# Kim-Dongjun/Soft-Truncation

Measured on AMD Instinct MI355X. Metric: training images/sec (DDPM++ CIFAR-10 32x32), higher is better.
Workload: dtype f32; 1 GPU; DDPM++ (VP) CIFAR-10 32x32, configs/vp/CIFAR10/ddpmpp_nll_st.py (BASELINE configs[1]); per_gpu_batch=128, global_batch=128, parallelism=dp1

## Files before the change

### soft-truncation_amd/csrc/conv.hip

```cpp
#include "igemm.h"
#include "split.h"
#include "stk_fp16.h"
#include "stk_fp16_train.h"

namespace {

using igemm::Cfg;
using igemm::MnMajor;
using igemm::keep_if;
using igemm::strip_row;

typedef __attribute__((address_space(1))) float gfloat;

struct ConvP {
  const float* x1; const float* x2; int C1, C2;
  const float* w; int w_layout;
  const float* bias; const float* temb; int temb_stride; const float* res; float inv_div; int use_div;
  float* y;
  const float* dy; float* dx1; float* dx2; float beta1, beta2, alpha;
  float* part; long part_stride;
  int N, H, W, Cin, Cout, OH, OW, KH, KW, stride, pad, sshift;
  int HW, OHW, taps;
  int ohw_shift, ow_shift;
};
// ... 630 lines not shown
#pragma unroll
      for (int t = 0; t < 9; ++t) v[u][t] = src[(long)(z + u) * stride + (long)t * CC];
#pragma unroll
    for (int u = 0; u < 4; ++u)
#pragma unroll
      for (int t = 0; t < 9; ++t) acc[t] += v[u][t];
  }
  for (; z < splits; ++z)
#pragma unroll
    for (int t = 0; t < 9; ++t) acc[t] += src[(long)z * stride + (long)t * CC];
#pragma unroll
  for (int t = 0; t < 9; ++t) s[threadIdx.x * 9 + t] = alpha * acc[t];
  __syncthreads();
  const long base = q0 * 9, end = CC * 9;
#pragma unroll
  for (int k = 0; k < 9; ++k) {
    const long i = base + k * 256 + threadIdx.x;
    if (i < end) dw[i] += s[k * 256 + threadIdx.x];
  }
}

template <int COLS>
__global__ __launch_bounds__(256) void wgrad9_kernel(ConvP p, int tiles_m, int tiles_n, int k_per_split) {
  constexpr int ROWS = 32 / COLS, TW = COLS + 2, TH = ROWS + 2, TSZ = TH * TW;
  constexpr int XS = TSZ | 1;
  constexpr int LDA = 129;
  constexpr int NX = (32 * TSZ + 255) / 256;
  constexpr int NA = 16;
  __shared__ float lds[32 * LDA + 32 * XS];
  float* As = lds;
  float* Xs = lds + 32 * LDA;

  const int tid = threadIdx.x, lane = tid & 63, wid = tid >> 6;
  const int fk = lane >> 5, fc = lane & 31;
  const int id = xcd_remap(blockIdx.x, gridDim.x);
  const int tn = id % tiles_n;
  const int rest = id / tiles_n;
  const int tm = rest % tiles_m, zs = rest / tiles_m;
  const int m0 = tm * 128, n0 = tn * 32;
  const int K = p.N * p.OHW;
  const int k_begin = zs * k_per_split;
  const int k_end = min(K, k_begin + k_per_split);

  const int mrow = m0 + (tid >> 5), cout_hi = p.Cout - 1;
  unsigned okrowsA = 0;
#pragma unroll
  for (int i = 0; i < NA; ++i) okrowsA |= (mrow + 8 * i < p.Cout ? 1u : 0u) << i;
  const int cin_hi = p.Cin - 1;
  floatx16 acc[9];
#pragma unroll
  for (int t = 0; t < 9; ++t)
#pragma unroll
    for (int e = 0; e < 16; ++e) acc[t][e] = 0.f;

  float ra[NA], rx[NX];
  unsigned okmA = 0, okmX = 0;
  auto load = [&](int k0) {
    const int k = k0 + (tid & 31);
    const bool kv = k < K;
    int b, ohw;
    split_pixel(p, kv ? k : 0, b, ohw);
    const int abase = b * p.Cout * p.OHW + ohw;
    okmA = kv ? okrowsA : 0u;
#pragma unroll
    for (int i = 0; i < NA; ++i) ra[i] = p.dy[abase + min(mrow + 8 * i, cout_hi) * p.OHW];
    int b0, ohw0, oy0, ox0;
    split_pixel(p, k0, b0, ohw0);
    split_row(p, ohw0, oy0, ox0);
    const int xbase = b0 * p.Cin * p.HW + (oy0 - 1) * p.W + (ox0 - 1);
    okmX = 0;
#pragma unroll
    for (int i = 0; i < NX; ++i) {
      const int e = tid + 256 * i;
      const int ci = e / TSZ, rem = e - ci * TSZ;
      const int lr = rem / TW, lc = rem - lr * TW;
      const int iy = oy0 - 1 + lr, ix = ox0 - 1 + lc;
      const bool ok = e < 32 * TSZ && n0 + ci < p.Cin && iy >= 0 && iy < p.H && ix >= 0 && ix < p.W;
      rx[i] = p.x1[ok ? xbase + min(n0 + ci, cin_hi) * p.HW + lr * p.W + lc : 0];
      okmX |= (ok ? 1u : 0u) << i;
    }
  };
  auto store = [&]() {
#pragma unroll
    for (int i = 0; i < NA; ++i) As[(tid & 31) * LDA + (tid >> 5) + 8 * i] = keep_if(ra[i], okmA, i);
#pragma unroll
    for (int i = 0; i < NX; ++i) {
      const int e = tid + 256 * i;
      const int ci = e / TSZ, rem = e - ci * TSZ;
      if (e < 32 * TSZ) Xs[ci * XS + rem] = keep_if(rx[i], okmX, i);
    }
  };

  if (k_begin < k_end) load(k_begin);
  const float* arow = As + fk * LDA + wid * 32 + fc;
  const float* xrow = Xs + fc * XS + fk;
  for (int k0 = k_begin; k0 < k_end; k0 += 32) {
    store();
    __syncthreads();
    if (k0 + 32 < k_end) load(k0 + 32);
#pragma unroll
    for (int ks = 0; ks < 16; ++ks) {
      const float a = arow[2 * ks * LDA];
      constexpr int dummy = 0; (void)dummy;
      const int loc = ((2 * ks) / COLS) * TW + ((2 * ks) % COLS);
      float bv[9];
#pragma unroll
      for (int t = 0; t < 9; ++t) bv[t] = xrow[loc + (t / 3) * TW + (t % 3)];
#pragma unroll
      for (int t = 0; t < 9; ++t) acc[t] = __builtin_amdgcn_mfma_f32_32x32x2f32(a, bv[t], acc[t], 0, 0, 0);
    }
    __syncthreads();
  }

  float* slab = p.part + (long)zs * p.part_stride;
  const int n = n0 + fc;
  if (n < p.Cin) {
#pragma unroll
    for (int t = 0; t < 9; ++t)
#pragma unroll
      for (int e = 0; e < 16; ++e) {
        const int m = m0 + wid * 32 + strip_row(e) + 4 * fk;
        if (m < p.Cout) slab[((long)t * p.Cout + m) * p.Cin + n] = acc[t][e];
      }
  }
}

struct GemmP {
  const float* A; long sam, sak, sab;
  const float* B; long sbk, sbn, sbb;
  float* C; long scm, scn, scb;
  const float* bias; int bias_mode;
  int M, N, K;
  float alpha, beta;
};
template <class C, bool K_CONTIG>
struct GA {
  RowChunk<C::BM, C::KC, C::LDA> rc;
  MnStrided<C::BM, C::KC, C::LDA> ms;
  __device__ void init(const GemmP& p, int m0, int tid, int zb) {
    const float* base = p.A + (long)zb * p.sab;
    if (K_CONTIG) rc.init(base, p.sam, m0, p.M, p.K, tid);
    else ms.init(base, p.sam, p.sak, m0, p.M, p.K, tid);
  }
  __device__ void load(const GemmP&, int k0, float (&r)[C::NA]) {
    if (K_CONTIG) rc.load(k0, r); else ms.load(k0, r);
  }
  __device__ void store(const float (&r)[C::NA], float* t) {
    if (K_CONTIG) rc.store(r, t); else ms.store(r, t);
  }
};
template <class C, bool K_CONTIG>
struct GB {
  RowChunk<C::BN, C::KC, C::LDB> rc;
  MnStrided<C::BN, C::KC, C::LDB> ms;
  __device__ void init(const GemmP& p, int n0, int tid, int zb) {
    const float* base = p.B + (long)zb * p.sbb;
    if (K_CONTIG) rc.init(base, p.sbn, n0, p.N, p.K, tid);
    else ms.init(base, p.sbn, p.sbk, n0, p.N, p.K, tid);
  }
  __device__ void load(const GemmP&, int k0, float (&r)[C::NB]) {
    if (K_CONTIG) rc.load(k0, r); else ms.load(k0, r);
  }
  __device__ void store(const float (&r)[C::NB], float* t) {
    if (K_CONTIG) rc.store(r, t); else ms.store(r, t);
  }
};
struct EpGemm {
  float* base;
  __device__ void init(const GemmP& p, int zb, int) { base = p.C + (long)zb * p.scb; }
  __device__ void col(const GemmP&, int) {}
  __device__ void strip(const GemmP& p, int mbase, int M, bool nok, int n, const floatx16& acc) {
    float old[16];
    if (p.beta != 0.f) {
#pragma unroll
      for (int e = 0; e < 16; ++e) {
        const int m = mbase + strip_row(e);
        const bool ok = nok && m < M;
        old[e] = base[ok ? (long)m * p.scm + (long)n * p.scn : 0];
      }
    }
#pragma unroll
    for (int e = 0; e < 16; ++e) {
      const int m = mbase + strip_row(e);
      if (nok && m < M) {
        float v = p.alpha * acc[e];
        if (p.bias_mode == 1) v += p.bias[m];
        else if (p.bias_mode == 2) v += p.bias[n];
        base[(long)m * p.scm + (long)n * p.scn] = (p.beta != 0.f ? p.beta * old[e] : 0.f) + v;
      }
    }
  }
};

inline bool use_big_tile(int M, long N, int z) {
  const long t = (long)stk_cdiv(M, 128) * stk_cdiv(N, 128) * z;
  return M >= 96 && N >= 96 && t >= 192;
}

template <class C, class P, class AL, class BL, class EP>
int launch(const P& p, int M, long Nl, int K, int k_per_split, int splits, int batch, hipStream_t s,
           bool flat = false) {
  if (Nl > 0x7fffffffL) return STK_EUNSUPPORTED;
  const int N = (int)Nl;
  const int tm = stk_cdiv(M, C::BM), tn = stk_cdiv(N, C::BN);
  if (flat) {
    const long total = (long)tm * tn * splits * batch;
    if (total > 0x7fffffffL) return STK_EUNSUPPORTED;
    hipLaunchKernelGGL((igemm::kernel<C, P, AL, BL, EP>), dim3((unsigned)total), dim3(256), 0, s, p, M, N, K, tm, tn,
                       k_per_split, batch);
  } else {
    dim3 grid((unsigned)(tm * tn), (unsigned)splits, (unsigned)batch);
    hipLaunchKernelGGL((igemm::kernel<C, P, AL, BL, EP>), grid, dim3(256), 0, s, p, M, N, K, tm, tn, k_per_split, 0);
  }
  STK_CHECK_LAUNCH();
  return STK_OK;
}

inline int fill_common(ConvP& p, int N, int H, int W, int C1, int C2, int Cout, int OH, int OW, int KH, int KW,
                       int stride, int pad) {
  if (N <= 0 || H <= 0 || W <= 0 || C1 <= 0 || C2 < 0 || Cout <= 0 || OH <= 0 || OW <= 0) return STK_EINVAL;
  if (!((KH == 3 && KW == 3) || (KH == 1 && KW == 1))) return STK_EUNSUPPORTED;
  if (stride != 1 && stride != 2) return STK_EUNSUPPORTED;
  const long lim = 0x7fffffffL;
  if ((long)N * (C1 > C2 ? C1 : C2) * H * W >= lim || (long)N * Cout * OH * OW >= lim) return STK_EUNSUPPORTED;
  p.N = N; p.H = H; p.W = W; p.C1 = C1; p.C2 = C2; p.Cin = C1 + C2; p.Cout = Cout; p.OH = OH; p.OW = OW;
  p.KH = KH; p.KW = KW; p.stride = stride; p.pad = pad; p.sshift = stride == 2 ? 1 : 0;
  p.HW = H * W; p.OHW = OH * OW; p.taps = KH * KW;
  p.ohw_shift = -1; p.ow_shift = -1;
  for (int sft = 0; sft < 31; ++sft) {
    if ((1 << sft) == p.OHW) p.ohw_shift = sft;
    if ((1 << sft) == p.OW) p.ow_shift = sft;
  }
  return STK_OK;
}

struct SplitPlan { int ok; int splits; int chunks_per_split; long slab; int t64; int gps; };
inline SplitPlan split_plan(const ConvP& p, int Kc, int S1, int S2, int M, long Ng) {
  SplitPlan r = {0, 1, 0, 0, 0, 0};
  const long big = (long)p.N * p.HW * 4 * (S1 > S2 ? S1 : S2);
  const bool geom = (p.taps == 9 && p.pad == 1) || (p.taps == 1 && p.pad == 0);
  if (!(big < 0x7fffffffL && geom && p.stride == 1 && p.OH == p.H && p.OW == p.W && Kc % 32 == 0 &&
        (S2 == 0 || S1 % 32 == 0) && M >= 96 && Ng <= 0x7fffffffL))
    return r;
  const long tiles = (long)stk_cdiv(M, 128) * stk_cdiv(Ng, 128);
  const int nch = p.taps * (Kc / 32);
  r.chunks_per_split = nch;
  if (tiles >= 192) { r.ok = 1; return r; }
  static const long target = [] { const char* e = getenv("STK_KSPLIT_WGS"); return e && atol(e) > 0 ? atol(e) : 512L; }();
  constexpr long minch = 12;
  long splits = target / tiles;
  const long mc = p.taps == 9 ? minch : (minch < 6 ? minch : 6);
  if (splits > nch / mc) splits = nch / mc;
  if ((tiles < 16 && p.taps != 9) || splits < 2) return r;
  r.chunks_per_split = (int)((nch + splits - 1) / splits);
  r.splits = (nch + r.chunks_per_split - 1) / r.chunks_per_split;
  r.slab = (long)M * Ng;
  r.ok = 1;
  return r;
}
inline SplitPlan fwd_split_plan(const ConvP& p) { return split_plan(p, p.Cin, p.C1, p.C2, p.Cout, (long)p.N * p.OHW); }
inline SplitPlan dgrad_split_plan(const ConvP& p) { return split_plan(p, p.Cout, p.Cout, 0, p.Cin, (long)p.N * p.HW); }
struct SplitWs { long xpart, part, bytes; };
inline long align256(long v) { return (v + 255) & ~255L; }
inline SplitWs split_ws(const SplitPlan& r, int M, int Kc, int taps) {
  SplitWs o;
  o.xpart = align256(x2::wp_bytes(M, Kc, taps));
  o.part = align256(o.xpart + 2L * x2::NPART * 4);
  o.bytes = r.ok ? 255 + o.part + (r.splits > 1 ? r.splits * r.slab * 4 : 0) : 0;
  return o;
}
inline void split_weight_strides(const ConvP& p, int dgrad, long& sm, long& sk) {
  if (p.w_layout == 0) { sm = dgrad ? p.taps : (long)p.Cin * p.taps; sk = dgrad ? (long)p.Cin * p.taps : p.taps; }
  else { sm = dgrad ? p.Cout : 1; sk = dgrad ? 1 : p.Cout; }
}
inline SplitPlan x1_plan(const SplitPlan& r, int nch1) {
  SplitPlan r1 = r;
  r1.chunks_per_split = (nch1 + r.splits - 1) / r.splits;
  r1.splits = (nch1 + r1.chunks_per_split - 1) / r1.chunks_per_split;
  return r1;
}

struct SplitGemm {
  ConvP p; x2::Src q; int M, Ng, tm, tn, nch, chunks_per_split; const float* xpart; int nx;
  bool dual, planes, halo; dim3 grid; hipStream_t s;
};
template <class E, int TAPS>
void split_gemm_taps(const SplitGemm& g) {
  constexpr bool X1 = is_x1<E>::value;
  if (!g.planes) {
    using A1 = std::conditional_t<X1, x2::ActLoader16<false, TAPS>, x2::ActLoader<false, TAPS>>;
    using A2 = std::conditional_t<X1, x2::ActLoader16<true, TAPS>, x2::ActLoader<true, TAPS>>;
    if (g.dual) hipLaunchKernelGGL((x2::gemm_kernel<A2, E>), g.grid, dim3(256), 0, g.s, g.p, g.q, g.M, g.Ng, g.tm, g.tn, g.nch,
                                   g.chunks_per_split, g.xpart, g.nx);
    else hipLaunchKernelGGL((x2::gemm_kernel<A1, E>), g.grid, dim3(256), 0, g.s, g.p, g.q, g.M, g.Ng, g.tm, g.tn, g.nch,
                            g.chunks_per_split, g.xpart, g.nx);
  } else if (g.halo) {
    if (g.p.W == 64)
      hipLaunchKernelGGL((x2d::gemm_halo_kernel<64, E, 1>), g.grid, dim3(256), 0, g.s, g.p, g.q, g.M, g.Ng, g.tm, g.tn, g.nch / 9, g.xpart, g.nx);
    else if (g.p.W == 32)
      hipLaunchKernelGGL((x2d::gemm_halo_kernel<32, E, 1>), g.grid, dim3(256), 0, g.s, g.p, g.q, g.M, g.Ng, g.tm, g.tn, g.nch / 9, g.xpart, g.nx);
    else
      hipLaunchKernelGGL((x2d::gemm_halo_kernel<16, E, 1>), g.grid, dim3(256), 0, g.s, g.p, g.q, g.M, g.Ng, g.tm, g.tn, g.nch / 9, g.xpart, g.nx);
  } else {
    hipLaunchKernelGGL((x2d::gemm_kernel<TAPS, 128, E>), g.grid, dim3(256), 0, g.s, g.p, g.q, g.M, g.Ng, g.tm, g.tn, g.nch,
                       g.chunks_per_split, g.xpart, g.nx);
  }
}
template <class E>
void split_gemm(const SplitGemm& g) {
  if (g.p.taps == 9) split_gemm_taps<E, 9>(g);
  else split_gemm_taps<E, 1>(g);
}

template <class EP>
int launch_split(ConvP p, const SplitPlan& r0, const float* s1, int S1, const float* s2, int S2, int M, long Ng, int dgrad,
                 void* ws, hipStream_t s, const void* wp_ready, float* amax, const void* planes, const float* planes_amax,
                 bool amax_valid, bool x1) {
  x2::Src q;
  q.s1 = s1; q.s2 = S2 > 0 ? s2 : s1; q.S1 = S1; q.S2 = S2; q.Kc = S1 + S2; q.Mpad = x2::pad128(M); q.taps = p.taps;
  q.pl = static_cast<const unsigned char*>(planes); q.pl_stride = planes ? pl::plane_bytes(p.N, S1, p.HW) : 0;
  const SplitWs lay = split_ws(r0, M, q.Kc, p.taps);
  unsigned char* base = reinterpret_cast<unsigned char*>(((uintptr_t)ws + 255) & ~(uintptr_t)255);
  float* xpart = reinterpret_cast<float*>(base + lay.xpart);
  p.part = reinterpret_cast<float*>(base + lay.part);
  p.part_stride = r0.slab;
  if (amax) xpart = amax + (dgrad ? 2 * x2::NPART : 0);
  if (planes) {
    xpart = const_cast<float*>(planes_amax);
  } else if (!(amax_valid && amax)) {
    hipLaunchKernelGGL(x2::amax_partial_kernel, dim3(x2::NPART), dim3(x2::AMAX_THREADS), 0, s, s1, (long)p.N * S1 * p.HW, xpart);
    if (S2 > 0)
      hipLaunchKernelGGL(x2::amax_partial_kernel, dim3(x2::NPART), dim3(x2::AMAX_THREADS), 0, s, s2, (long)p.N * S2 * p.HW,
                         xpart + x2::NPART);
    STK_CHECK_LAUNCH();
  }
  if (wp_ready) {
    q.wp = static_cast<const unsigned short*>(wp_ready);
  } else {
    x2::WprepDesc one = {};
    one.w = p.w; one.wp = base; one.M = M; one.Kc = q.Kc; one.Mpad = q.Mpad;
    one.taps = p.taps; one.flip = dgrad;
    split_weight_strides(p, dgrad, one.sm, one.sk);
    hipLaunchKernelGGL(x2::wamax_kernel, dim3(x2::WPART, 1), dim3(256), 0, s, nullptr, one);
    hipLaunchKernelGGL(x2::wprep_kernel, dim3((unsigned)stk_cdiv((long)q.Mpad * q.Kc, 256L)), dim3(256), 0, s, nullptr, one);
    STK_CHECK_LAUNCH();
    q.wp = reinterpret_cast<const unsigned short*>(base);
  }
  const int nch = planes && x1 ? p.taps * ((q.Kc / x2::KC + 1) / 2) : p.taps * (q.Kc / x2::KC);
  const SplitPlan r = planes && x1 ? x1_plan(r0, nch) : r0;
  SplitGemm g = {p, q, M, (int)Ng, q.Mpad / 128, stk_cdiv((int)Ng, 128), nch, r.chunks_per_split, xpart,
                 S2 > 0 ? 2 * x2::NPART : x2::NPART, S2 > 0, planes != nullptr, planes && x2d::halo_ok(p, p.taps, r0.splits),
                 dim3(), s};
  g.grid = dim3((unsigned)(g.tm * g.tn * r.splits));
  if (r0.splits == 1) {
    if (x1) split_gemm<OneProduct<EP>>(g);
    else split_gemm<EP>(g);
    STK_CHECK_LAUNCH();
    return STK_OK;
  }
  if (x1) split_gemm<OneProduct<EpSlab>>(g);
  else split_gemm<EpSlab>(g);
  STK_CHECK_LAUNCH();
  launch_slab_sum(p, r.splits, M, Ng, dgrad, s);
  STK_CHECK_LAUNCH();
  return STK_OK;
}

struct SplitWgradPlan { int ok; int splits; int chunks_per_split; long slab; int rows3; };
inline SplitWgradPlan split_wgrad_plan(int C1, int C2, int N, int Cout, int H, int W, int OH, int OW, int KH, int KW,
                                       int stride, int pad) {
  SplitWgradPlan q = {0, 0, 0, 0, 0};
  const int Cin = C1 + C2;
  const long K = (long)N * H * W;
  const int cmax = Cout > C1 ? (Cout > C2 ? Cout : C2) : (C1 > C2 ? C1 : C2);
  if (K * cmax * 4 >= 0x7fffffffL || (C2 > 0 && C1 % 32)) return q;
  const bool pow2 = (W & (W - 1)) == 0 && ((H * W) & (H * W - 1)) == 0;
  const bool geom = (KH == 3 && KW == 3 && pad == 1) || (KH == 1 && KW == 1 && pad == 0);
  if (!geom || stride != 1 || OH != H || OW != W || !pow2 || W < 4 || H * W < 16 || Cin < 64 || Cout < 64 ||
      K > 0x7fffffffL || K % 32)
    return q;
  const int taps = KH * KW;
  q.rows3 = (taps == 9 && W >= 8 && (C2 == 0 || C1 % 16 == 0)) ? 1 : 0;
  const long tiles = q.rows3 ? 3L * stk_cdiv(Cout, 128) * stk_cdiv(Cin, 64)
                             : (long)taps * stk_cdiv(Cout, 128) * stk_cdiv(Cin, 128);
  if (taps == 1 && tiles < 2) return q;
  const long chunks = K / 32;
  constexpr long w1_wgs = 256;
  long splits = (taps == 1 && tiles < 6 ? w1_wgs : 512) / tiles;
  if (splits > chunks / 8) splits = chunks / 8;
  if (splits < 1) splits = 1;
  q.chunks_per_split = (int)((chunks + splits - 1) / splits);
  q.splits = (int)((chunks + q.chunks_per_split - 1) / q.chunks_per_split);
  q.slab = (long)Cout * Cin * taps;
  q.ok = 1;
  return q;
}
template <int FORM>
void launch_x2w(const x2w::Args& a, int W, dim3 grid, hipStream_t s) {
  const dim3 block(256 * (FORM & 15));
  if (W >= 32) hipLaunchKernelGGL((x2w::wgrad_kernel<32, FORM>), grid, block, 0, s, a);
  else if (W == 16) hipLaunchKernelGGL((x2w::wgrad_kernel<16, FORM>), grid, block, 0, s, a);
  else if (W == 8) hipLaunchKernelGGL((x2w::wgrad_kernel<8, FORM>), grid, block, 0, s, a);
  else hipLaunchKernelGGL((x2w::wgrad_kernel<4, FORM>), grid, block, 0, s, a);
}
struct WgemmArgs {
  ConvP p; int tm, tn, nch, chunks_per_split; const float* dyp; const float* xp; int nx; dim3 grid; hipStream_t s;
};
template <bool X1, class BL>
void launch_wgemm_rows(const WgemmArgs& g) {
  using AL = std::conditional_t<X1, x2::RowsU16<false, false>, x2::RowsU<false, false>>;
  using E = std::conditional_t<X1, OneProduct<EpWgrad>, EpWgrad>;
  hipLaunchKernelGGL((x2::wgemm_kernel<AL, BL, E, !X1>), g.grid, dim3(256), 0, g.s, g.p, g.p.Cout, g.p.Cin, g.tm, g.tn, g.nch,
                     g.chunks_per_split, g.p.taps, g.dyp, g.xp, g.nx);
}
template <bool X1, bool DUAL>
void launch_wgemm_src(const WgemmArgs& g) {
  if (g.p.taps == 1)
    launch_wgemm_rows<X1, std::conditional_t<X1, x2::RowsU16<true, DUAL>, x2::RowsU<true, DUAL>>>(g);
  else if (g.p.W >= 16)
    launch_wgemm_rows<X1, std::conditional_t<X1, x2::RowsB16<DUAL, 16>, x2::RowsB<DUAL, 16>>>(g);
  else if (g.p.W == 8)
    launch_wgemm_rows<X1, std::conditional_t<X1, x2::RowsB16<DUAL, 8>, x2::RowsB<DUAL, 8>>>(g);
  else
    launch_wgemm_rows<X1, std::conditional_t<X1, x2::RowsB16<DUAL, 4>, x2::RowsB<DUAL, 4>>>(g);
}
template <bool X1>
void launch_wgemm(const WgemmArgs& g) {
  if (g.p.C2 > 0) launch_wgemm_src<X1, true>(g);
  else launch_wgemm_src<X1, false>(g);
}

struct WgradPlan { int big; int splits; int k_per_split; long slab; int mode9; };
inline int wgrad9_cols(int OH, int OW, int KH, int KW) {
  if (KH != 3 || KW != 3 || ((long)OH * OW) % 32 != 0) return 0;
  if (OW % 32 == 0) return 32;
  if (OW == 16 || OW == 8) return OW;
  return 0;
}
inline WgradPlan wgrad_plan(int Cin, int N, int Cout, int OH, int OW, int KH, int KW, bool allow9 = true) {
  WgradPlan q;
  q.mode9 = allow9 ? wgrad9_cols(OH, OW, KH, KW) : 0;
  if (q.mode9) {
    const long K = (long)N * OH * OW;
    const long tiles = (long)stk_cdiv(Cout, 128) * stk_cdiv(Cin, 32);
    const long chunks = K / 32;
    long splits = 256 / tiles;
    if (splits > chunks / 16) splits = chunks / 16;
    if (splits < 1) splits = 1;
    const long cps = (chunks + splits - 1) / splits;
    q.big = 1;
    q.k_per_split = (int)(cps * 32);
    q.splits = (int)((K + q.k_per_split - 1) / q.k_per_split);
    q.slab = (long)Cout * Cin * 9;
    return q;
  }
  const int taps = KH * KW;
  const long K = (long)N * OH * OW;
  const long tiles128 = (long)stk_cdiv(Cout, 128) * stk_cdiv(Cin, 128) * taps;
  q.big = (Cout >= 96 && Cin >= 96 && tiles128 >= 9) ? 1 : 0;
  const int T = q.big ? 128 : 64;
  const long tiles = (long)stk_cdiv(Cout, T) * stk_cdiv(Cin, T) * taps;
  const long chunks = (K + 31) / 32;
  long splits = (512 + tiles - 1) / tiles;
  if (splits > chunks / 16) splits = chunks / 16;
  if (splits < 1) splits = 1;
  const long cps = (chunks + splits - 1) / splits;
  q.k_per_split = (int)(cps * 32);
  q.splits = (int)((K + q.k_per_split - 1) / q.k_per_split);
  q.slab = (long)Cout * Cin * taps;
  return q;
}

}

extern "C" {

static int fwd_impl(const float* x1, int C1, const float* x2, int C2, const float* w, int w_layout,
                    const float* bias, const float* temb, int temb_stride, const float* res, float out_div,
                    float* y, int N, int H, int W, int Cout, int OH, int OW, int KH, int KW, int stride, int pad,
                    const void* wp, float* amax, void* ws, long ws_bytes, void* stream, bool x_rec_valid, bool f16x1) {
  if (!x1 || !w || !y || (C2 > 0 && !x2) || out_div == 0.f || (w_layout != 0 && w_layout != 1) ||
      (w_layout == 1 && (KH != 1 || KW != 1)))
    return STK_EINVAL;
  ConvP p = {};
  int rc = fill_common(p, N, H, W, C1, C2, Cout, OH, OW, KH, KW, stride, pad);
  if (rc) return rc;
  p.x1 = x1; p.x2 = C2 > 0 ? x2 : x1; p.w = w; p.w_layout = w_layout; p.bias = bias; p.temb = temb;
  p.temb_stride = temb_stride; p.res = res; p.inv_div = 1.f / out_div; p.use_div = out_div != 1.f; p.y = y;
  const int K = p.Cin * p.taps;
  const long Ng = (long)N * p.OHW;
  const bool big = use_big_tile(Cout, Ng, 1);
  hipStream_t s = (hipStream_t)stream;
  if (thin::geometry_ok(p) && Ng <= 0x7fffffffL) {
    const unsigned nblk = (unsigned)stk_cdiv(Ng, 256L);
    if (C2 == 0 && p.Cin <= 4) {
      thin::Args a = {x1, w, (long)p.Cin * p.taps, (long)p.taps, 0, p.Cin, Cout, p.taps, 0};
      const dim3 grid(nblk, (unsigned)stk_cdiv(Cout, thin::OB));
      if (p.taps == 9) hipLaunchKernelGGL((thin::thin_in_kernel<9>), grid, dim3(256), 0, s, p, a);
      else hipLaunchKernelGGL((thin::thin_in_kernel<1>), grid, dim3(256), 0, s, p, a);
      STK_CHECK_LAUNCH();
      return STK_OK;
    }
    if (Cout <= 4) {
      const unsigned nblk64 = (unsigned)stk_cdiv(Ng, 64L);
      if (p.taps == 9) hipLaunchKernelGGL((thin::thin_out_kernel<9>), dim3(nblk64), dim3(256), 0, s, p, Cout);
      else hipLaunchKernelGGL((thin::thin_out_kernel<1>), dim3(nblk64), dim3(256), 0, s, p, Cout);
      STK_CHECK_LAUNCH();
      return STK_OK;
    }
  }
  const SplitPlan xr = fwd_split_plan(p);
  if (ws && xr.ok && ws_bytes >= split_ws(xr, Cout, p.Cin, p.taps).bytes)
    return launch_split<EpFwd>(p, xr, x1, C1, x2, C2, Cout, Ng, 0, ws, s, wp, amax, nullptr, nullptr, x_rec_valid, f16x1);
  if (wp) return STK_EINVAL;
  if (p.taps == 9) {
    using CB = Cfg<128, 128, 36>; using CS = Cfg<64, 64, 36>;
    if (C2 > 0) {
      if (big) return launch<CB, ConvP, AFwdK<CB>, BFwd<CB, 9, true>, EpFwd>(p, Cout, Ng, K, K, 1, 1, s);
      return launch<CS, ConvP, AFwdK<CS>, BFwd<CS, 9, true>, EpFwd>(p, Cout, Ng, K, K, 1, 1, s);
    }
    if (big) return launch<CB, ConvP, AFwdK<CB>, BFwd<CB, 9, false>, EpFwd>(p, Cout, Ng, K, K, 1, 1, s);
    return launch<CS, ConvP, AFwdK<CS>, BFwd<CS, 9, false>, EpFwd>(p, Cout, Ng, K, K, 1, 1, s);
  }
  using CB = Cfg<128, 128, 32>; using CS = Cfg<64, 64, 32>;
  if (w_layout == 0) {
    if (K % 8 == 0) {
      if (big) return launch<CB, ConvP, AFwdK<CB>, BFwd<CB, 1, true>, EpFwd>(p, Cout, Ng, K, K, 1, 1, s);
      return launch<CS, ConvP, AFwdK<CS>, BFwd<CS, 1, true>, EpFwd>(p, Cout, Ng, K, K, 1, 1, s);
    }
    return launch<CS, ConvP, AFwdGen<CS>, BFwd<CS, 1, true>, EpFwd>(p, Cout, Ng, K, K, 1, 1, s);
  }
  if (big) return launch<CB, ConvP, AFwdNin<CB>, BFwd<CB, 1, true>, EpFwd>(p, Cout, Ng, K, K, 1, 1, s);
  return launch<CS, ConvP, AFwdNin<CS>, BFwd<CS, 1, true>, EpFwd>(p, Cout, Ng, K, K, 1, 1, s);
}

int stk_conv2d_fwd_f32(const float* x1, int C1, const float* x2, int C2, const float* w, int w_layout,
                       const float* bias, const float* temb, int temb_stride, const float* res, float out_div,
                       float* y, int N, int H, int W, int Cout, int OH, int OW, int KH, int KW, int stride, int pad,
                       void* ws, long ws_bytes, void* stream) {
  return stk_conv2d_fwd_wp_f32(x1, C1, x2, C2, w, w_layout, bias, temb, temb_stride, res, out_div, y, N, H, W, Cout, OH, OW,
                               KH, KW, stride, pad, nullptr, nullptr, ws, ws_bytes, stream);
}

int stk_conv2d_fwd_wp_f32(const float* x1, int C1, const float* x2, int C2, const float* w, int w_layout,
                          const float* bias, const float* temb, int temb_stride, const float* res, float out_div,
                          float* y, int N, int H, int W, int Cout, int OH, int OW, int KH, int KW, int stride, int pad,
                          const void* wp, float* amax, void* ws, long ws_bytes, void* stream) {
  return fwd_impl(x1, C1, x2, C2, w, w_layout, bias, temb, temb_stride, res, out_div, y, N, H, W, Cout, OH, OW, KH, KW, stride,
                  pad, wp, amax, ws, ws_bytes, stream, false, false);
}

int stk_conv2d_fwd_rec_f32(const float* x1, int C1, const float* x2, int C2, const float* w, int w_layout,
                           const float* bias, const float* temb, int temb_stride, const float* res, float out_div,
                           float* y, int N, int H, int W, int Cout, int OH, int OW, int KH, int KW, int stride, int pad,
                           const void* wp, float* amax, void* ws, long ws_bytes, void* stream) {
  if (!amax) return STK_EINVAL;
  return fwd_impl(x1, C1, x2, C2, w, w_layout, bias, temb, temb_stride, res, out_div, y, N, H, W, Cout, OH, OW, KH, KW, stride,
                  pad, wp, amax, ws, ws_bytes, stream, true, false);
}

int stk_conv2d_fwd_wp_f16x1(const float* x1, int C1, const float* x2, int C2, const float* w, int w_layout,
                            const float* bias, const float* temb, int temb_stride, const float* res, float out_div,
                            float* y, int N, int H, int W, int Cout, int OH, int OW, int KH, int KW, int stride, int pad,
                            const void* wp, float* amax, void* ws, long ws_bytes, void* stream) {
  return fwd_impl(x1, C1, x2, C2, w, w_layout, bias, temb, temb_stride, res, out_div, y, N, H, W, Cout, OH, OW, KH, KW, stride,
                  pad, wp, amax, ws, ws_bytes, stream, false, true);
}

int stk_conv2d_fwd_rec_f16x1(const float* x1, int C1, const float* x2, int C2, const float* w, int w_layout,
                             const float* bias, const float* temb, int temb_stride, const float* res, float out_div,
                             float* y, int N, int H, int W, int Cout, int OH, int OW, int KH, int KW, int stride, int pad,
                             const void* wp, float* amax, void* ws, long ws_bytes, void* stream) {
  if (!amax) return STK_EINVAL;
  return fwd_impl(x1, C1, x2, C2, w, w_layout, bias, temb, temb_stride, res, out_div, y, N, H, W, Cout, OH, OW, KH, KW, stride,
                  pad, wp, amax, ws, ws_bytes, stream, true, true);
}

static int dgrad_impl(const float* dy, const float* w, int w_layout, float* dx1, int C1, float beta1, float* dx2,
                      int C2, float beta2, float alpha, int N, int H, int W, int Cout, int OH, int OW, int KH,
                      int KW, int stride, int pad, const void* wp, float* amax, void* ws, long ws_bytes,
                      void* stream, bool dy_rec_valid, bool f16x1) {
  if (!dy || !w || (!dx1 && !dx2) || (w_layout != 0 && w_layout != 1) || (w_layout == 1 && (KH != 1 || KW != 1)))
    return STK_EINVAL;
  ConvP p = {};
  int rc = fill_common(p, N, H, W, C1, C2, Cout, OH, OW, KH, KW, stride, pad);
  if (rc) return rc;
  p.dy = dy; p.w = w; p.w_layout = w_layout; p.dx1 = dx1; p.dx2 = C2 > 0 ? dx2 : nullptr;
  p.beta1 = beta1; p.beta2 = beta2; p.alpha = alpha;
  const int Cin = p.Cin;
  const int K = Cout * p.taps;
  const long Ng = (long)N * p.HW;
  const bool big = use_big_tile(Cin, Ng, 1);
  hipStream_t s = (hipStream_t)stream;
  if (thin::geometry_ok(p) && Cout <= 4 && Ng <= 0x7fffffffL) {
    thin::Args a = {dy, w, (long)p.taps, (long)Cin * p.taps, 1, Cout, Cin, p.taps, 1};
    const dim3 grid((unsigned)stk_cdiv(Ng, 256L), (unsigned)stk_cdiv(Cin, thin::OB));
    if (p.taps == 9) hipLaunchKernelGGL((thin::thin_in_kernel<9>), grid, dim3(256), 0, s, p, a);
    else hipLaunchKernelGGL((thin::thin_in_kernel<1>), grid, dim3(256), 0, s, p, a);
    STK_CHECK_LAUNCH();
    return STK_OK;
  }
  const SplitPlan xr = dgrad_split_plan(p);
  if (ws && xr.ok && ws_bytes >= split_ws(xr, Cin, Cout, p.taps).bytes)
    return launch_split<EpDgrad>(p, xr, dy, Cout, nullptr, 0, Cin, Ng, 1, ws, s, wp, amax, nullptr, nullptr, dy_rec_valid, f16x1);
  if (wp) return STK_EINVAL;
  if (p.taps == 9) {
    using CB = Cfg<128, 128, 36>; using CS = Cfg<64, 64, 36>;
    if (big) return launch<CB, ConvP, ADgrad9<CB>, BDgrad<CB, 9>, EpDgrad>(p, Cin, Ng, K, K, 1, 1, s);
// ... 464 lines not shown
```

### soft-truncation_amd/csrc/conv_x2d.h

```cpp
#pragma once

namespace x2d {

using x2::KC;
typedef __attribute__((address_space(3))) void lds_void;

template <int TN>
struct Geo {
  static constexpr int A_PLANE = 128 * 64, A_BYTES = 2 * A_PLANE;
  static constexpr int B_PLANE = TN * 64, B_BYTES = 2 * B_PLANE;
  static constexpr int LDS = A_BYTES + B_BYTES;
  static constexpr int NJ = TN / 64;
  static constexpr int BBLK = TN / 64;
};

__device__ __forceinline__ void dma16(__amdgpu_buffer_rsrc_t rs, unsigned char* dst, unsigned voff, unsigned soff) {
  __builtin_amdgcn_raw_ptr_buffer_load_lds(rs, (lds_void*)dst, 16, (int)voff, (int)soff, 0, 0);
}

template <int TAPS, int TN, class EP, int NBUF = 1, int ABL = 0>
__global__ __launch_bounds__(256, 2) void gemm_kernel(ConvP p, x2::Src q, int M, int Nn, int tiles_m, int tiles_n,
                                                      int nchunks_total, int chunks_per_split,
                                                      const float* __restrict__ xpart, int nxpart) {
  using G = Geo<TN>;
  constexpr bool X1 = is_x1<EP>::value;
  __shared__ __attribute__((aligned(1024))) unsigned char lds[G::LDS * NBUF];
  unsigned char* const As = lds;
  unsigned char* const Bs = lds + G::A_BYTES;
  const int tid = threadIdx.x;
  const int lane = tid & 63, wid = __builtin_amdgcn_readfirstlane(tid >> 6);
  __shared__ float red_amax[4];
  x2::LateAmax xmax;
  xmax.load(xpart, nxpart, tid);
  const float sw = x2::weight_scale(q.wp);
  const int ntiles = tiles_m * tiles_n;
  const int id = xcd_remap(blockIdx.x, gridDim.x);
  const int tile = id % ntiles, zs = id / ntiles;
  const int tm = tile % tiles_m, tn = tile / tiles_m;
  const int m0 = tm * 128, n0 = tn * TN;
  const int c_begin = zs * chunks_per_split;
  const int c_last = min(nchunks_total, c_begin + chunks_per_split) - 1;

  const unsigned seg_src = (unsigned)((lane & 3) ^ ((lane >> 4) & 3)) * 16u;
  const unsigned a_plane2 = (unsigned)q.taps * q.Mpad * q.Kc * 2u;
  const unsigned a_chunk2 = (unsigned)q.Mpad * KC * 2u;
  const __amdgpu_buffer_rsrc_t a_rs = x2::make_rsrc(reinterpret_cast<const unsigned char*>(q.wp) + x2::HEADER, 2L * a_plane2);
  const unsigned a_voff = (unsigned)(m0 + 32 * wid + (lane >> 2)) * 64u + seg_src;
  const __amdgpu_buffer_rsrc_t b_rs = x2::make_rsrc(q.pl, 2L * q.pl_stride);
  const unsigned b_ps = (unsigned)q.pl_stride;
  const int Cb = q.Kc >> 5;
  unsigned b_base[G::BBLK], b_mask[G::BBLK];
  {
#pragma unroll
    for (int jb = 0; jb < G::BBLK; ++jb) {
      const int n = n0 + (TN / 4) * wid + 16 * jb + (lane >> 2);
      b_mask[jb] = 0; b_base[jb] = 0;
      if (n < Nn) {
        const int b = n / p.HW, hw = n - b * p.HW;
        const int y = hw / p.W, x = hw - y * p.W;
        if (TAPS == 1) b_mask[jb] = 1u;
#pragma unroll
        for (int t = 0; t < (TAPS == 9 ? 9 : 0); ++t) {
          const int iy = y + t / 3 - 1, ix = x + t % 3 - 1;
          if (iy >= 0 && iy < p.H && ix >= 0 && ix < p.W) b_mask[jb] |= 1u << t;
        }
        b_base[jb] = ((unsigned)(b * Cb) * p.HW + hw) * 64u + seg_src;
      }
    }
  }
  auto stage = [&](int c, int buf = 0) {
    const int cc = TAPS == 9 ? c / 9 : c, tap = c - cc * TAPS;
    const unsigned a_soff = (unsigned)c * a_chunk2;
    unsigned char* const As = lds + buf * G::LDS;
    unsigned char* const Bs = As + G::A_BYTES;
    if (X1) {
#pragma unroll
      for (int s = 0; s < 2; ++s) {
        const unsigned dead = (2 * cc + s >= Cb) ? 0x80000000u : 0u;
#pragma unroll
        for (int h = 0; h < 2; ++h)
          dma16(a_rs, As + s * G::A_PLANE + (32 * wid + 16 * h) * 64, (a_voff + h * 1024u) | dead,
                (unsigned)((2 * cc + s) * TAPS + tap) * a_chunk2);
      }
    } else if (!(ABL & 2) || c == c_begin) {
#pragma unroll
    for (int s = 0; s < 2; ++s)
#pragma unroll
      for (int h = 0; h < 2; ++h)
        dma16(a_rs, As + s * G::A_PLANE + (32 * wid + 16 * h) * 64, a_voff + h * 1024u, a_soff + s * a_plane2);
    }
    const int shift = TAPS == 9 ? ((tap / 3 - 1) * p.W + (tap % 3 - 1)) * 64 : 0;
    const unsigned b_soff = (unsigned)cc * (unsigned)p.HW * 64u;
    if ((ABL & 1) && tap != 0) return;
#pragma unroll
    for (int jb = 0; jb < G::BBLK; ++jb) {
      const unsigned dead = (((b_mask[jb] >> tap) & 1u) ^ 1u) << 31;
      const unsigned vo = (b_base[jb] + (unsigned)shift) | dead;
#pragma unroll
      for (int s = 0; s < 2; ++s) {
        if (X1)
          dma16(b_rs, Bs + s * G::B_PLANE + ((TN / 4) * wid + 16 * jb) * 64, vo | (2 * cc + s >= Cb ? 0x80000000u : 0u),
                (unsigned)(2 * cc + s) * (unsigned)p.HW * 64u);
        else
          dma16(b_rs, Bs + s * G::B_PLANE + ((TN / 4) * wid + 16 * jb) * 64, vo, b_soff + s * b_ps);
      }
    }
  };

  EP ep;
  ep.preload(p, m0, n0, TN, M, Nn, tid);

  floatx16 acc[2][G::NJ];
#pragma unroll
  for (int i = 0; i < 2; ++i)
#pragma unroll
    for (int j = 0; j < G::NJ; ++j)
#pragma unroll
      for (int e = 0; e < 16; ++e) acc[i][j][e] = 0.f;

  const int wm0 = (wid & 1) * 64, wn0 = (wid >> 1) * (TN / 2);
  const int fk = lane >> 5, fc = lane & 31;
  const int fsw = (fc >> 2) & 3;
  const unsigned char* a_rd = As + (wm0 + fc) * 64;
  const unsigned char* b_rd = Bs + (wn0 + fc) * 64;
  const int ko0 = ((0 + fk) ^ fsw) * 16, ko1 = ((2 + fk) ^ fsw) * 16;

#define STK_D_FRAGS_AT(KO, OFF)                                                                           \
  _Pragma("unroll") for (int s = 0; s < 2; ++s) {                                                          \
    _Pragma("unroll") for (int i = 0; i < 2; ++i)                                                           \
      a[i][s] = *reinterpret_cast<const halfx8*>(a_rd + (OFF) + s * G::A_PLANE + i * 32 * 64 + (KO));      \
    _Pragma("unroll") for (int j = 0; j < G::NJ; ++j)                                                       \
      b[j][s] = *reinterpret_cast<const halfx8*>(b_rd + (OFF) + s * G::B_PLANE + j * 32 * 64 + (KO));      \
  }
#define STK_D_FRAGS(KO) STK_D_FRAGS_AT(KO, 0)
  constexpr int SA[3] = {1, 0, 0}, SB[3] = {0, 1, 0};
  constexpr int NPR = X1 ? 2 : 3;
#define STK_D_MFMAS                                                                                        \
  _Pragma("unroll") for (int pr = 0; pr < NPR; ++pr) _Pragma("unroll") for (int i = 0; i < 2; ++i)           \
    _Pragma("unroll") for (int j = 0; j < G::NJ; ++j) {                                                     \
      acc[i][j] = __builtin_amdgcn_mfma_f32_32x32x16_f16(a[i][X1 ? pr : SA[pr]], b[j][X1 ? pr : SB[pr]], acc[i][j], 0, 0, 0); \
    }

  halfx8 a[2][2], b[G::NJ][2];
  stage(c_begin);
  if constexpr (NBUF == 2) {
    int cur = 0;
    for (int c = c_begin; c <= c_last; ++c) {
      asm volatile("s_waitcnt vmcnt(0)" ::: "memory");
      __syncthreads();
      if (c < c_last) stage(c + 1, cur ^ 1);
      const int off = cur * G::LDS;
      STK_D_FRAGS_AT(ko0, off)
      STK_D_MFMAS
      STK_D_FRAGS_AT(ko1, off)
      STK_D_MFMAS
      cur ^= 1;
    }
  } else {
    for (int c = c_begin; c <= c_last; ++c) {
      asm volatile("s_waitcnt vmcnt(0)" ::: "memory");
      __syncthreads();
      if (!(ABL & 4) || c == c_begin) { STK_D_FRAGS(ko0) }
      STK_D_MFMAS
      if (!(ABL & 4) || c == c_begin) { STK_D_FRAGS(ko1) }
      __syncthreads();
      if (c < c_last) stage(c + 1);
      STK_D_MFMAS
    }
  }
#undef STK_D_MFMAS
#undef STK_D_FRAGS
#undef STK_D_FRAGS_AT

  const float unscale = 1.f / (sw * x2::pow2_scale_of(xmax.reduce(red_amax, tid)));
  ep.stage(lds, tid);
  ep.init(p, 0, zs);
#pragma unroll
  for (int j = 0; j < G::NJ; ++j) {
    const int n = n0 + wn0 + j * 32 + fc;
    const bool nok = n < Nn;
    ep.col(p, nok ? n : 0);
#pragma unroll
    for (int i = 0; i < 2; ++i) {
#pragma unroll
      for (int e = 0; e < 16; ++e) acc[i][j][e] *= unscale;
      ep.strip(p, m0 + wm0 + i * 32 + 4 * fk, M, nok, nok ? n : 0, acc[i][j]);
    }
  }
  ep.finish(p, lds, tid);
}

template <int W, class EP, int NB>
__global__ __launch_bounds__(256, 2) void gemm_halo_kernel(ConvP p, x2::Src q, int M, int Nn, int tiles_m, int tiles_n,
                                                           int ngroups, const float* __restrict__ xpart, int nxpart) {
  constexpr int TN = 128, R = TN / W, TP = W + 2, HR = (R + 2) * TP, NI = (HR + 15) / 16, HRP = NI * 16;
  constexpr bool X1 = is_x1<EP>::value;
  constexpr int A_PLANE = 128 * 64, A_BYTES = 2 * A_PLANE, B_PLANE = HRP * 64, B_BYTES = 2 * B_PLANE;
  constexpr int NK = (NI + 3) / 4;
  static_assert(NB == 1 || 2 * NK <= 8, "the B pieces of a group are issued one per chunk over taps 0..7");
  __shared__ __attribute__((aligned(1024))) unsigned char lds[A_BYTES + NB * B_BYTES];
  unsigned char* const As = lds;
  unsigned char* const Bs = lds + A_BYTES;
  const int tid = threadIdx.x;
  const int lane = tid & 63, wid = __builtin_amdgcn_readfirstlane(tid >> 6);
  __shared__ float red_amax[4];
  x2::LateAmax xmax;
  xmax.load(xpart, nxpart, threadIdx.x);
  const float sw = x2::weight_scale(q.wp);
  const int ntiles = tiles_m * tiles_n;
  const int id = xcd_remap(blockIdx.x, gridDim.x);
  const int tile = id % ntiles;
  const int tm = tile % tiles_m, tn = tile / tiles_m;
  const int m0 = tm * 128, n0 = tn * TN;
  const int nchunks = 9 * ngroups;

  const unsigned seg_src = (unsigned)((lane & 3) ^ ((lane >> 4) & 3)) * 16u;
  const unsigned a_plane2 = (unsigned)q.taps * q.Mpad * q.Kc * 2u;
  const unsigned a_chunk2 = (unsigned)q.Mpad * KC * 2u;
  const __amdgpu_buffer_rsrc_t a_rs = x2::make_rsrc(reinterpret_cast<const unsigned char*>(q.wp) + x2::HEADER, 2L * a_plane2);
  const unsigned a_voff = (unsigned)(m0 + 32 * wid + (lane >> 2)) * 64u + seg_src;
  const __amdgpu_buffer_rsrc_t b_rs = x2::make_rsrc(q.pl, 2L * q.pl_stride);
  const unsigned b_ps = (unsigned)q.pl_stride;
  const int Cb = q.Kc >> 5;
  unsigned b_voff[NK];
  {
    const int b = n0 / p.HW, hw0 = n0 - b * p.HW, y0 = hw0 / p.W, x0 = hw0 - y0 * p.W;
#pragma unroll
    for (int k = 0; k < NK; ++k) {
      const int row = 16 * (wid + 4 * k) + (lane >> 2);
      const int ty = row / TP, tx = row - ty * TP;
      const int y = y0 - 1 + ty, x = x0 + tx - 1;
      const bool ok = row < HR && y >= 0 && y < p.H && x >= 0 && x < p.W;
      b_voff[k] = ok ? ((unsigned)(b * Cb) * p.HW + (unsigned)(y * p.W + x)) * 64u + seg_src : 0x80000000u;
    }
  }
  auto stage_a = [&](int c) {
    if (X1) {
      const int cc = c / 9, tap = c - 9 * cc;
#pragma unroll
      for (int s = 0; s < 2; ++s) {
        const unsigned dead = (2 * cc + s >= Cb) ? 0x80000000u : 0u;
#pragma unroll
        for (int h = 0; h < 2; ++h)
          dma16(a_rs, As + s * A_PLANE + (32 * wid + 16 * h) * 64, (a_voff + h * 1024u) | dead,
                (unsigned)((2 * cc + s) * 9 + tap) * a_chunk2);
      }
      return;
    }
    const unsigned a_soff = (unsigned)c * a_chunk2;
#pragma unroll
    for (int s = 0; s < 2; ++s)
#pragma unroll
      for (int h = 0; h < 2; ++h)
        dma16(a_rs, As + s * A_PLANE + (32 * wid + 16 * h) * 64, a_voff + h * 1024u, a_soff + s * a_plane2);
  };
  auto stage_b = [&](int cc, int buf, int k, int s) {
    if (wid + 4 * k >= NI) return;
    if (X1) {
      dma16(b_rs, Bs + buf * B_BYTES + s * B_PLANE + (wid + 4 * k) * 1024, b_voff[k] | (2 * cc + s >= Cb ? 0x80000000u : 0u),
            (unsigned)(2 * cc + s) * (unsigned)p.HW * 64u);
      return;
    }
    dma16(b_rs, Bs + buf * B_BYTES + s * B_PLANE + (wid + 4 * k) * 1024, b_voff[k],
          (unsigned)cc * (unsigned)p.HW * 64u + s * b_ps);
  };

  EP ep;
  ep.preload(p, m0, n0, TN, M, Nn, tid);

  floatx16 acc[2][2];
#pragma unroll
  for (int i = 0; i < 2; ++i)
#pragma unroll
    for (int j = 0; j < 2; ++j)
#pragma unroll
      for (int e = 0; e < 16; ++e) acc[i][j][e] = 0.f;

  const int wm0 = (wid & 1) * 64, wn0 = (wid >> 1) * 64;
  const int fk = lane >> 5, fc = lane & 31;
  const int fsw = (fc >> 2) & 3;
  const unsigned char* a_rd = As + (wm0 + fc) * 64;
  const int ka0 = ((0 + fk) ^ fsw) * 16, ka1 = ((2 + fk) ^ fsw) * 16;
  int b_row[2];
#pragma unroll
  for (int j = 0; j < 2; ++j) {
    const int pt = wn0 + 32 * j + fc;
    b_row[j] = (pt / W + 1) * TP + (pt % W) + 1;
  }

  halfx8 a[2][2], b[2][2];
  constexpr int SA[3] = {1, 0, 0}, SB[3] = {0, 1, 0};
  constexpr int NPR = X1 ? 2 : 3;
#define STK_H_MFMAS                                                                                        \
  _Pragma("unroll") for (int pr = 0; pr < NPR; ++pr) _Pragma("unroll") for (int i = 0; i < 2; ++i)           \
    _Pragma("unroll") for (int j = 0; j < 2; ++j) {                                                         \
      acc[i][j] = __builtin_amdgcn_mfma_f32_32x32x16_f16(a[i][X1 ? pr : SA[pr]], b[j][X1 ? pr : SB[pr]], acc[i][j], 0, 0, 0); \
    }
#define STK_H_FRAGS(KA, KSEG)                                                                              \
  _Pragma("unroll") for (int s = 0; s < 2; ++s) {                                                          \
    _Pragma("unroll") for (int i = 0; i < 2; ++i)                                                           \
      a[i][s] = *reinterpret_cast<const halfx8*>(a_rd + s * A_PLANE + i * 32 * 64 + (KA));                 \
    _Pragma("unroll") for (int j = 0; j < 2; ++j)                                                           \
      b[j][s] = *reinterpret_cast<const halfx8*>(bbase + s * B_PLANE + brow[j] * 64 + ((((KSEG) + fk) ^ (brow[j] >> 2)) & 3) * 16); \
  }

#pragma unroll
  for (int k = 0; k < NK; ++k)
#pragma unroll
    for (int s = 0; s < 2; ++s) stage_b(0, 0, k, s);
  stage_a(0);
  int c = 0;
  for (int cc = 0; cc < ngroups; ++cc) {
    const unsigned char* bbase = Bs + (NB == 2 ? (cc & 1) * B_BYTES : 0);
    const bool more = cc + 1 < ngroups;
#pragma unroll
    for (int tap = 0; tap < 9; ++tap, ++c) {
      const int toff = (tap / 3 - 1) * TP + (tap % 3 - 1);
      int brow[2] = {b_row[0] + toff, b_row[1] + toff};
      asm volatile("s_waitcnt vmcnt(0)" ::: "memory");
      __syncthreads();
      STK_H_FRAGS(ka0, 0)
      STK_H_MFMAS
      STK_H_FRAGS(ka1, 2)
      __syncthreads();
      if (c + 1 < nchunks) stage_a(c + 1);
      if (NB == 2) {
        if (tap < 2 * NK && more) stage_b(cc + 1, (cc + 1) & 1, tap >> 1, tap & 1);
      } else if (tap == 8 && more) {
#pragma unroll
        for (int k = 0; k < NK; ++k)
#pragma unroll
          for (int s = 0; s < 2; ++s) stage_b(cc + 1, 0, k, s);
      }
      STK_H_MFMAS
    }
  }
#undef STK_H_MFMAS
#undef STK_H_FRAGS

  const float unscale = 1.f / (sw * x2::pow2_scale_of(xmax.reduce(red_amax, tid)));
  ep.stage(lds, tid);
  ep.init(p, 0, 0);
#pragma unroll
  for (int j = 0; j < 2; ++j) {
    const int n = n0 + wn0 + j * 32 + fc;
    ep.col(p, n);
#pragma unroll
    for (int i = 0; i < 2; ++i) {
#pragma unroll
      for (int e = 0; e < 16; ++e) acc[i][j][e] *= unscale;
      ep.strip(p, m0 + wm0 + i * 32 + 4 * fk, M, true, n, acc[i][j]);
    }
  }
  ep.finish(p, lds, tid);
}

inline int halo_cols(int W) { return (W == 16 || W == 32 || W == 64) ? W : 0; }
inline bool halo_ok(const ConvP& p, int taps, int splits) {
  return taps == 9 && splits == 1 && halo_cols(p.W) != 0 && p.HW % 128 == 0 && p.H * p.W == p.HW;
}

}
```

Measured before the change: 3510 images/s.

## Add three-deep LDS ring pipeline for small-grid implicit-GEMM conv kernels

Adds a triple-buffered LDS ring to the x2d GEMM kernel that keeps two stages of buffer-to-LDS DMA in flight, using a counted vmcnt wait instead of draining all loads each chunk. The launcher picks ring depth 3 when the grid has at most 256 workgroups (else the single-buffer path), clamped by chunk count and an environment cap. The aim is to hide global-load latency in under-filled grids, at the cost of halving occupancy (launch bounds of 1) and more LDS per workgroup. It also adds an inline-asm DMA path with hand-built resource descriptors that manipulates m0 directly.

```diff
diff --git a/soft-truncation_amd/csrc/conv.hip b/soft-truncation_amd/csrc/conv.hip
--- a/soft-truncation_amd/csrc/conv.hip
+++ b/soft-truncation_amd/csrc/conv.hip
@@ -956,8 +956,20 @@
     else
       hipLaunchKernelGGL((x2d::gemm_halo_kernel<16, E, 1>), g.grid, dim3(256), 0, g.s, g.p, g.q, g.M, g.Ng, g.tm, g.tn, g.nch / 9, g.xpart, g.nx);
   } else {
-    hipLaunchKernelGGL((x2d::gemm_kernel<TAPS, 128, E>), g.grid, dim3(256), 0, g.s, g.p, g.q, g.M, g.Ng, g.tm, g.tn, g.nch,
-                       g.chunks_per_split, g.xpart, g.nx);
+    const int chunks = g.chunks_per_split < g.nch ? g.chunks_per_split : g.nch;
+    switch (x2d::ring_depth((long)g.grid.x, chunks)) {
+      case 3:
+        hipLaunchKernelGGL((x2d::gemm_kernel<TAPS, 128, E, 3>), g.grid, dim3(256), 0, g.s, g.p, g.q, g.M, g.Ng, g.tm, g.tn, g.nch,
+                           g.chunks_per_split, g.xpart, g.nx);
+        break;
+      case 2:
+        hipLaunchKernelGGL((x2d::gemm_kernel<TAPS, 128, E, 2>), g.grid, dim3(256), 0, g.s, g.p, g.q, g.M, g.Ng, g.tm, g.tn, g.nch,
+                           g.chunks_per_split, g.xpart, g.nx);
+        break;
+      default:
+        hipLaunchKernelGGL((x2d::gemm_kernel<TAPS, 128, E>), g.grid, dim3(256), 0, g.s, g.p, g.q, g.M, g.Ng, g.tm, g.tn, g.nch,
+                           g.chunks_per_split, g.xpart, g.nx);
+    }
   }
 }
 template <class E>
diff --git a/soft-truncation_amd/csrc/conv_x2d.h b/soft-truncation_amd/csrc/conv_x2d.h
--- a/soft-truncation_amd/csrc/conv_x2d.h
+++ b/soft-truncation_amd/csrc/conv_x2d.h
@@ -18,12 +18,25 @@
   __builtin_amdgcn_raw_ptr_buffer_load_lds(rs, (lds_void*)dst, 16, (int)voff, (int)soff, 0, 0);
 }
 
+__device__ __forceinline__ u32x4 rsrc_words(const void* base, long bytes) {
+  const unsigned long p = reinterpret_cast<unsigned long>(base);
+  return u32x4{(unsigned)p, (unsigned)(p >> 32) & 0xffffu, (unsigned)bytes, 0x00020000u};
+}
+__device__ __forceinline__ void dma16(u32x4 rs, unsigned char* dst, unsigned voff, unsigned soff) {
+  const unsigned lds_addr = (unsigned)(unsigned long)(lds_void*)dst;
+  unsigned keep;
+  asm volatile("s_mov_b32 %0, m0\n\ts_mov_b32 m0, %1\n\ts_nop 4\n\tbuffer_load_dwordx4 %2, %3, %4 offen lds\n\ts_mov_b32 m0, %0"
+               : "=&s"(keep) : "s"(lds_addr), "v"(voff), "s"(rs), "s"(soff) : "memory");
+}
+
 template <int TAPS, int TN, class EP, int NBUF = 1, int ABL = 0>
-__global__ __launch_bounds__(256, 2) void gemm_kernel(ConvP p, x2::Src q, int M, int Nn, int tiles_m, int tiles_n,
+__global__ __launch_bounds__(256, NBUF == 3 ? 1 : 2) void gemm_kernel(ConvP p, x2::Src q, int M, int Nn, int tiles_m, int tiles_n,
                                                       int nchunks_total, int chunks_per_split,
                                                       const float* __restrict__ xpart, int nxpart) {
   using G = Geo<TN>;
   constexpr bool X1 = is_x1<EP>::value;
+  static_assert(NBUF >= 1 && NBUF <= 3 && (NBUF == 3 ? 1 : 2) * (G::LDS * NBUF + 1024) <= 160 * 1024,
+                "ring images of the workgroups meant to share a CU (two; one with three images) exceed its 160 KB of LDS");
   __shared__ __attribute__((aligned(1024))) unsigned char lds[G::LDS * NBUF];
   unsigned char* const As = lds;
   unsigned char* const Bs = lds + G::A_BYTES;
@@ -44,9 +57,10 @@
   const unsigned seg_src = (unsigned)((lane & 3) ^ ((lane >> 4) & 3)) * 16u;
   const unsigned a_plane2 = (unsigned)q.taps * q.Mpad * q.Kc * 2u;
   const unsigned a_chunk2 = (unsigned)q.Mpad * KC * 2u;
-  const __amdgpu_buffer_rsrc_t a_rs = x2::make_rsrc(reinterpret_cast<const unsigned char*>(q.wp) + x2::HEADER, 2L * a_plane2);
+  auto rsrc = [](const void* base, long bytes) { if constexpr (NBUF >= 2) return rsrc_words(base, bytes); else return x2::make_rsrc(base, bytes); };
+  const auto a_rs = rsrc(reinterpret_cast<const unsigned char*>(q.wp) + x2::HEADER, 2L * a_plane2);
   const unsigned a_voff = (unsigned)(m0 + 32 * wid + (lane >> 2)) * 64u + seg_src;
-  const __amdgpu_buffer_rsrc_t b_rs = x2::make_rsrc(q.pl, 2L * q.pl_stride);
+  const auto b_rs = rsrc(q.pl, 2L * q.pl_stride);
   const unsigned b_ps = (unsigned)q.pl_stride;
   const int Cb = q.Kc >> 5;
   unsigned b_base[G::BBLK], b_mask[G::BBLK];
@@ -143,18 +157,22 @@
 
   halfx8 a[2][2], b[G::NJ][2];
   stage(c_begin);
-  if constexpr (NBUF == 2) {
+  if constexpr (NBUF >= 2) {
+    constexpr int AHEAD = NBUF - 1, NDMA = 4 + 2 * G::BBLK;
+    static_assert(NBUF <= 3 && NDMA == 8, "the counted wait below is written for one stage() of 8 DMA instructions in flight");
+    if (NBUF == 3 && c_begin < c_last) stage(c_begin + 1, 1);
     int cur = 0;
     for (int c = c_begin; c <= c_last; ++c) {
-      asm volatile("s_waitcnt vmcnt(0)" ::: "memory");
-      __syncthreads();
-      if (c < c_last) stage(c + 1, cur ^ 1);
+      if (NBUF == 3 && c < c_last) asm volatile("s_waitcnt vmcnt(8)" ::: "memory");
+      else asm volatile("s_waitcnt vmcnt(0)" ::: "memory");
+      __syncthreads();
+      if (c + AHEAD <= c_last) stage(c + AHEAD, cur == 0 ? NBUF - 1 : cur - 1);
       const int off = cur * G::LDS;
       STK_D_FRAGS_AT(ko0, off)
       STK_D_MFMAS
       STK_D_FRAGS_AT(ko1, off)
       STK_D_MFMAS
-      cur ^= 1;
+      cur = cur + 1 == NBUF ? 0 : cur + 1;
     }
   } else {
     for (int c = c_begin; c <= c_last; ++c) {
@@ -188,6 +206,14 @@
     }
   }
   ep.finish(p, lds, tid);
+}
+
+inline int ring_cap() { static const int v = [] { const char* e = getenv("STK_X2D_RING"); const int n = e ? atoi(e) : 3; return n < 1 || n > 3 ? 3 : n; }(); return v; }
+inline int ring_depth(long workgroups, int chunks) {
+  int d = workgroups <= 256 ? 3 : 1;
+  if (d > chunks) d = chunks;
+  if (d > ring_cap()) d = ring_cap();
+  return d < 1 ? 1 : d;
 }
 
 template <int W, class EP, int NB>
```

Result: no change. 3504 images/s (-0.2%).
